# LiuShenLan/global_body_planner

Measured on AMD Instinct MI355X. Metric: valid extend-attempts/sec + time-to-first-solution, 1024×1024 rough_terrain, higher is better.
Workload: dtype f64; 1 GPU; config 3: synth-rough-1024, 262,144-attempt batch per GPU, isValidStateActionPair[Reverse] 50/50; terrain=synth-rough-1024, batch_per_gpu=262144, global_batch=262144, seed=20251018, kernel=persistent, waves=2, adaptive=False, terrain_storage=f32, parallelism=shard1 (no collective on the data path)

## Files before the change

global_body_planner_amd/csrc/gbp_engine.hip:

```cpp
#pragma clang fp contract(off)

#include <hip/hip_runtime.h>
#include <stdint.h>
#include <string.h>

#include <cstring>

#include <algorithm>
#include <cmath>
#include <mutex>
#include <new>
#include <vector>

#include "gbp.h"
#include "gbp_device.h"
#include "gbp_lane.h"
#include "gbp_um_order.h"
#include "gbp_internal.h"
#include "host/gbp_host_check.h"

using namespace gbp;

namespace {

// ... 53 lines not shown
    if (is_nan) is_nan[i] = r != 0 ? 1 : 0;
    if (ood) ood[i] = (!ok || r < 0) ? 1 : 0;
  }
}

template <class ZT>
__global__ void k_normal(TerrainView<ZT> T, int64_t n, const double *__restrict__ xy,
                         double *__restrict__ nrm, uint8_t *__restrict__ ood) {
  for (int64_t i = blockIdx.x * (int64_t)blockDim.x + threadIdx.x; i < n;
       i += (int64_t)gridDim.x * blockDim.x) {
    double v[3];
    const bool ok = surface_normal(T, xy[2 * i], xy[2 * i + 1], v);
    nrm[3 * i] = v[0];
    nrm[3 * i + 1] = v[1];
    nrm[3 * i + 2] = v[2];
    if (ood) ood[i] = ok ? 0 : 1;
  }
}

template <class ZT>
__global__ void k_valid_states(TerrainView<ZT> T, int64_t n, const double *__restrict__ states,
                               const uint8_t *__restrict__ phase, int phase_all,
                               uint8_t *__restrict__ valid, uint32_t *__restrict__ flags,
                               uint32_t *__restrict__ counts) {
  for (int64_t i = blockIdx.x * (int64_t)blockDim.x + threadIdx.x; i < n;
       i += (int64_t)gridDim.x * blockDim.x) {
    double s[8];
#pragma unroll
    for (int k = 0; k < 8; k++) s[k] = states[8 * i + k];
    Acc acc{0, 0, 0};
    const bool v = is_valid_state(T, s, phase ? phase[i] : phase_all, acc);
    if (valid) valid[i] = v;
    if (flags) flags[i] = acc.flags | (v ? GBP_F_VALID : 0u);
    if (counts) counts[i] = (acc.G & 0xFFFFu) | (acc.V << 16);
  }
}

extern __shared__ double gbp_smem[];

template <class ZT, bool ADAPTIVE, int W, int CM>
__global__ __launch_bounds__(256, W) void k_validate_direct(
    TerrainView<ZT> T0, int64_t n, const double *__restrict__ S, const double *__restrict__ A,
    const uint8_t *__restrict__ dir, int dir_all, uint8_t *__restrict__ valid,
    double *__restrict__ s_new, double *__restrict__ t_new, uint32_t *__restrict__ flags,
    uint32_t *__restrict__ counts) {
  const TerrainView<ZT> T = CM == 1 ? stage_coords(T0, gbp_smem) : T0;
  const int64_t i = blockIdx.x * (int64_t)blockDim.x + threadIdx.x;
  if (i >= n) return;
  double s[8], a[10], sn[8];
#pragma unroll
  for (int k = 0; k < 8; k++) s[k] = S[8 * i + k];
#pragma unroll
  for (int k = 0; k < 10; k++) a[k] = A[10 * i + k];
  double tn = 0;
  Acc acc{0, 0, 0};
  uint32_t f = 0;
  const int d = dir ? dir[i] : dir_all;
  const bool v = (d == GBP_FORWARD) ? pair_forward<ZT, ADAPTIVE>(T, s, a, sn, tn, acc, f)
                                    : pair_reverse<ZT, ADAPTIVE>(T, s, a, sn, tn, acc, f);
  f |= acc.flags | (v ? GBP_F_VALID : 0u);
  if (valid) valid[i] = v;
  if (s_new && (f & GBP_F_SNEW_SET)) {
#pragma unroll
    for (int k = 0; k < 8; k++) s_new[8 * i + k] = sn[k];
  }
  if (t_new && (f & GBP_F_TNEW_SET)) t_new[i] = tn;
  flags[i] = f;
  if (counts) counts[i] = (acc.G & 0xFFFFu) | (acc.V << 16);
}



struct SnewRec {
  int idx, kind;
  double p;
};
constexpr int SN_RING = 2 * 64;

#ifdef GBP_LOOP_PROF
constexpr int LP_N = 14;
__device__ unsigned long long gbp_loop_prof[8192 * LP_N];
#define LP_T(v) const unsigned long long v = __builtin_readcyclecounter()
#define LP_ADD(k, a, b) lp[k] += (b) - (a)
#else
#define LP_T(v)
#define LP_ADD(k, a, b)
#endif

[[maybe_unused]] constexpr int PF_MAX = 32;

inline size_t rows_bytes(int block, int pf) {
  const size_t nwv = (size_t)(block / WAVE);
  return sizeof(double) * SA_ROW * (size_t)(WAVE + pf) * nwv + sizeof(SnewRec) * SN_RING * nwv +
         sizeof(int) * ((nwv * (size_t)pf + 1) & ~(size_t)1);
}

__device__ __forceinline__ void row_to_lds(const double *S, const double *A, const uint8_t *dir,
                                           unsigned int i, double *row, int lane) {
  const unsigned int lds = __builtin_amdgcn_readfirstlane(
      (unsigned int)(uintptr_t)(__attribute__((address_space(3))) void *)row);
  const uint32_t *src = lane < 16 ? (const uint32_t *)(S + 8 * (size_t)i) + lane
                                  : (const uint32_t *)(A + 10 * (size_t)i) + (lane - 16);
  unsigned int keep;
  if (lane < 36)
    asm volatile("s_mov_b32 %0, m0\n\ts_mov_b32 m0, %2\n\ts_nop 0\n\t"
                 "global_load_lds_dword %1, off\n\ts_mov_b32 m0, %0"
                 : "=&s"(keep) : "v"(src), "s"(lds) : "memory");
  if (dir && lane == 36)
    asm volatile("s_mov_b32 %0, m0\n\ts_mov_b32 m0, %2\n\ts_nop 0\n\t"
                 "global_load_lds_ubyte %1, off\n\ts_mov_b32 m0, %0"
                 : "=&s"(keep) : "v"(dir + i), "s"(lds) : "memory");
}

template <class ZT, bool ADAPTIVE, int W, int CM, bool ONE>
__global__ __launch_bounds__(512, W) void k_validate_persistent(
    TerrainView<ZT> T0, int n, const double *__restrict__ S, const double *__restrict__ A,
    const uint8_t *__restrict__ dir, int dir_all, uint8_t *__restrict__ valid,
    double *__restrict__ s_new, double *__restrict__ t_new, uint32_t *__restrict__ flags,
    uint32_t *__restrict__ counts, const int *__restrict__ n_dev, int helpers, int xcd_map, int pf) {
#ifdef GBP_LOOP_PROF
  const unsigned long long lp_entry = __builtin_amdgcn_s_memrealtime();
#endif
  if (n_dev) n = *n_dev;
  const int lane = threadIdx.x & (WAVE - 1);
  const unsigned long long lt_mask = (1ull << lane) - 1ull;
  const int nwv = blockDim.x / WAVE, wv = __builtin_amdgcn_readfirstlane(threadIdx.x / WAVE);
  double *const SA = gbp_smem + (CM == 1 ? (T0.nx + T0.ny + 1) & ~1 : 0);
  double *const wave_rows = SA + (size_t)wv * (WAVE + pf) * SA_ROW;
  SnewRec *const ring = (SnewRec *)(SA + (size_t)nwv * (WAVE + pf) * SA_ROW) + wv * SN_RING;
  [[maybe_unused]] int *const Q = (int *)(ring + (nwv - wv) * SN_RING) + wv * pf;
  unsigned int cur, end;
  {
    const unsigned int waves = gridDim.x * (blockDim.x / WAVE);
    const unsigned int wg = (xcd_map && (gridDim.x & 7u) == 0)
                                ? (blockIdx.x & 7u) * (gridDim.x >> 3) + (blockIdx.x >> 3)
                                : blockIdx.x;
    const unsigned int wid = wg * (blockDim.x / WAVE) + wv;
    cur = __builtin_amdgcn_readfirstlane((unsigned int)(((unsigned long long)n * wid) / waves));
    end = __builtin_amdgcn_readfirstlane((unsigned int)(((unsigned long long)n * (wid + 1)) / waves));
  }
  auto load_row = [&](unsigned int i, double *r, int &d) {
    if (dir) d = dir[i];
#pragma unroll
    for (int k = 0; k < 8; k++) r[k] = S[8 * (size_t)i + k];
#pragma unroll
    for (int k = 0; k < 10; k++) r[8 + k] = A[10 * (size_t)i + k];
  };
#ifdef GBP_REFILL_WINDOW
  const unsigned int take0 = min(end - cur, (unsigned int)WAVE);
  double row0[18];
  int dir0 = dir_all;
  if ((unsigned int)lane < take0) load_row(cur + lane, row0, dir0);
#endif
  const TerrainView<ZT> T = CM == 1 ? stage_coords(T0, gbp_smem) : T0;
  int ring_n = 0;
  auto flush = [&](int cnt) {
    if (lane < cnt) {
      const SnewRec r = ring[lane];
      double sv[8], av[10], o[8];
#pragma unroll
      for (int k = 0; k < 8; k++) sv[k] = S[8 * (size_t)r.idx + k];
#pragma unroll
      for (int k = 0; k < 10; k++) av[k] = A[10 * (size_t)r.idx + k];
      sample_state(sv, av,
                   r.kind == SN_STANCE_S ? ST_FWD_STANCE
                                         : (r.kind == SN_FLIGHT_B ? ST_FWD_LAND : ST_REV_STANCE),
                   r.p, o);
#pragma unroll
      for (int k = 0; k < 8; k++) s_new[8 * (size_t)r.idx + k] = o[k];
    }
  };
  Lane L;
  int row = lane;
  L.s = wave_rows + row * SA_ROW;
  L.a = L.s + 8;
  L.stage = ST_IDLE;
  auto start = [&](unsigned int i, int d) {
    L.idx = (int)i;
    L.f = 0;
    L.acc = Acc{0, 0, 0};
    L.snew_kind = SN_NONE;
    L.tnew_set = 0;
    enter_stage(L, d == GBP_FORWARD ? ST_FWD_STANCE : ST_REV_FLIGHT);
  };
#ifdef GBP_REFILL_WINDOW
  unsigned int staged = 0, qh = 0;
  if (lane < pf) Q[lane] = WAVE + lane;
  if ((unsigned int)lane < take0) {
#pragma unroll
    for (int k = 0; k < 18; k++) L.s[k] = row0[k];
    start(cur + lane, dir0);
  }
  cur += take0;
#endif
#ifdef GBP_LOOP_PROF
  unsigned long long lp[LP_N] = {0, 0, 0, 0, 0, 0, 0, 0, 0, 0, 0, 0, 0, 0};
  lp[12] = lp_entry;
  lp[8] = __builtin_amdgcn_s_memrealtime();
  LP_T(lp_start);
#endif
  for (;;) {
    LP_T(t0);
    const bool need = L.stage == ST_IDLE;
    unsigned long long m = __ballot(need);
    if (m && cur < end) {
      const unsigned int take = min(end - cur, (unsigned int)__popcll(m));
      const unsigned int rank = (unsigned int)__popcll(m & lt_mask);
      const bool mine = need && rank < take;
      unsigned int ts = 0;
#ifdef GBP_REFILL_WINDOW
      ts = min(take, staged);
      if (ts) {
        asm volatile("s_waitcnt vmcnt(0)" ::: "memory");
        if (mine && rank < ts) {
          unsigned int p = qh + rank;
          p -= p >= (unsigned int)pf ? (unsigned int)pf : 0u;
          const int got = Q[p];
          Q[p] = row;
          row = got;
          L.s = wave_rows + row * SA_ROW;
          L.a = L.s + 8;
          start(cur + rank, dir ? ((const int *)L.s)[36] & 0xFF : dir_all);
        }
        qh += ts;
        qh -= qh >= (unsigned int)pf ? (unsigned int)pf : 0u;
        staged -= ts;
      }
#endif
      if (mine && rank >= ts) {
        double r[18];
        int d = dir_all;
        load_row(cur + rank, r, d);
#pragma unroll
        for (int k = 0; k < 18; k++) L.s[k] = r[k];
        start(cur + rank, d);
      }
      cur += take;
    }
#ifdef GBP_REFILL_WINDOW
    if (pf && min(end - cur, (unsigned int)pf) > staged) {
      const unsigned int want = min(end - cur, (unsigned int)pf);
      const int qv = Q[lane < pf ? lane : 0];
      for (unsigned int k = staged; k < want; k++) {
        unsigned int p = qh + k;
        p -= p >= (unsigned int)pf ? (unsigned int)pf : 0u;
        row_to_lds(S, A, dir, cur + k, wave_rows + __builtin_amdgcn_readlane(qv, p) * SA_ROW, lane);
      }
      staged = want;
    }
#endif
    const unsigned long long act = __ballot(L.stage != ST_IDLE);
    if (!act) break;
    LP_T(t1);
    LP_ADD(0, t0, t1);
#ifdef GBP_LOOP_PROF
    if (!lp[7]) lp[13] = __builtin_amdgcn_s_memrealtime();
#endif
    const bool owner = L.stage != ST_IDLE;
    asm volatile("" ::: "memory");
    const int n_act = __popcll(act);
    const bool tail = helpers && n_act < WAVE;
    int st = L.stage, slot = 0;
    const double *ps = L.s;
    double t_eval = owner ? stage_time(L) : 0.0;
    uint32_t vbase = L.acc.V;
    bool has = owner;
    if (tail) {
      const unsigned long long idle = ~act;
      const int j = __popcll(idle & lt_mask);
      const int src = owner ? lane : nth_set_bit(act, j % n_act);
      slot = owner ? 0 : 1 + j / n_act;
      ps = wave_rows + __shfl(row, src) * SA_ROW;
      st = __shfl(L.stage, src);
      double t = __shfl(L.t, src), ts = __shfl(L.ts, src);
      vbase = __shfl(L.acc.V, src);
      if (!owner) {
        has = true;
        for (int k = 0; k < slot && has; k++) has = advance_on_success<ADAPTIVE>(st, ps + 8, t, ts);
        t_eval = sample_time(st, ps + 8, t);
      }
    }
    LP_T(t2);
    LP_ADD(1, t1, t2);
    Acc acc_s{0, vbase + (uint32_t)slot, 0};
    bool ok = false;
    if (has) {
      double sc[8];
      sample_state(ps, ps + 8, st, t_eval, sc);
      ok = is_valid_state<ZT, CM, ONE>(T, sc, stage_phase(st), acc_s);
    }
    LP_T(t3);
    LP_ADD(2, t2, t3);
    bool decided = false;
    if (owner) {
      L.acc.G += acc_s.G;
      L.acc.V = acc_s.V;
      L.acc.flags |= acc_s.flags;
      decided = (acc_s.flags & GBP_F_LIMIT) ? true : transition<ADAPTIVE>(L, ok);
    }
    if (tail) {
      const unsigned long long idle = ~act;
      const int n_idle = WAVE - n_act;
      const int n_help = n_idle;
      const uint32_t w0 = (acc_s.flags & 0xFFFFu) | (ok ? 1u << 16 : 0u) | (has ? 1u << 17 : 0u) |
                          ((acc_s.V - (vbase + (uint32_t)slot)) << 18);
      const uint32_t w1 = acc_s.G;
      const int my_rank = __popcll(act & lt_mask);
      bool chain = owner && !decided && ok;
      const int kmax = (n_help + n_act - 1) / n_act;
      for (int k = 1; k <= kmax; k++) {
        if (!__ballot(chain)) break;
        const int j = (k - 1) * n_act + my_rank;
        const bool exists = owner && j < n_help;
        const int src = (exists && j < n_idle) ? nth_set_bit(idle, j) : lane;
        const uint32_t r0 = __shfl(w0, src), r1 = __shfl(w1, src);
        if (chain && exists && ((r0 >> 17) & 1u)) {
          L.acc.G += r1;
          L.acc.V += (r0 >> 18) & 1u;
          L.acc.flags |= r0 & 0xFFFFu;
          const bool okk = (r0 >> 16) & 1u;
          decided = (r0 & GBP_F_LIMIT) ? true : transition<ADAPTIVE>(L, okk);
          chain = !decided && okk;
        } else {
          chain = false;
        }
      }
    }
    asm volatile("" ::: "memory");
    LP_T(t4);
    LP_ADD(3, t3, t4);
#ifdef GBP_LOOP_PROF
    lp[6] += tail ? 1 : 0;
    lp[7] += 1;
#endif
    const bool fin = owner && decided;
    const bool queue = fin && s_new && L.snew_kind != SN_NONE;
    if (fin) {
      const size_t i = (size_t)L.idx;
      uint32_t f = L.f | L.acc.flags;
      if (L.snew_kind != SN_NONE) f |= GBP_F_SNEW_SET;
      if (L.tnew_set) f |= GBP_F_TNEW_SET;
      if (valid) valid[i] = (f & GBP_F_VALID) ? 1 : 0;
      if (t_new && L.tnew_set) t_new[i] = L.tnew;
      flags[i] = f;
      if (counts) counts[i] = (L.acc.G & 0xFFFFu) | (L.acc.V << 16);
    }
    const unsigned long long qm = __ballot(queue);
    if (qm) {
      if (queue) ring[ring_n + __popcll(qm & lt_mask)] = SnewRec{L.idx, L.snew_kind, L.snew_p};
      ring_n += __popcll(qm);
      if (ring_n >= WAVE) {
        flush(WAVE);
        ring_n -= WAVE;
        SnewRec r;
        if (lane < ring_n) r = ring[WAVE + lane];
        if (lane < ring_n) ring[lane] = r;
      }
    }
    if (fin) L.stage = ST_IDLE;
    LP_T(t5);
    LP_ADD(4, t4, t5);
  }
  if (ring_n) flush(ring_n);
#ifdef GBP_LOOP_PROF
  LP_T(lp_end);
  lp[5] = lp_end - lp_start;
  lp[9] = __builtin_amdgcn_s_memrealtime();
  {
    unsigned int hw;
    asm volatile("s_getreg_b32 %0, hwreg(HW_REG_HW_ID)" : "=s"(hw));
    lp[10] = hw;
    unsigned int xcc;
    asm volatile("s_getreg_b32 %0, hwreg(HW_REG_XCC_ID)" : "=s"(xcc));
    lp[11] = xcc;
  }
  const unsigned int gw = blockIdx.x * (blockDim.x / WAVE) + threadIdx.x / WAVE;
  if (lane == 0 && gw < 8192)
    for (int k = 0; k < LP_N; k++) gbp_loop_prof[LP_N * gw + k] = lp[k];
#endif
}

struct DirPair {
  double from[8], to[8];
};

template <class ZT>
__global__ void k_sample_states(TerrainView<ZT> T, int64_t n, uint64_t seed, uint64_t stream_id,
                                int64_t index_base, int require_phase, int max_tries,
                                double *__restrict__ states, int32_t *__restrict__ tries,
                                gbp_sampling cfg, DirPair dp) {
  for (int64_t i = blockIdx.x * (int64_t)blockDim.x + threadIdx.x; i < n;
       i += (int64_t)gridDim.x * blockDim.x) {
    double q[8];
    int got = -1;
    const int mt = max_tries > 0 ? max_tries : 1;
    for (int k = 0; k < mt; k++) {
      sample_state_cfg_try(T, cfg, dp.from, dp.to, seed, stream_id, index_base + i, k, q);
      if (require_phase < 0) { got = k + 1; break; }
      Acc acc{0, 0, 0};
      if (is_valid_state(T, q, require_phase, acc)) { got = k + 1; break; }
    }
#pragma unroll
    for (int k = 0; k < 8; k++) states[8 * i + k] = q[k];
    if (tries) tries[i] = got;
  }
}

__global__ void k_sample_actions(int64_t n, const double *__restrict__ normals, uint64_t seed,
                                 uint64_t stream_id, int64_t index_base,
                                 double *__restrict__ actions) {
  for (int64_t i = blockIdx.x * (int64_t)blockDim.x + threadIdx.x; i < n;
       i += (int64_t)gridDim.x * blockDim.x) {
    const double nv[3] = {normals[3 * i], normals[3 * i + 1], normals[3 * i + 2]};
    double a[10];
    sample_action(nv, seed, stream_id, index_base + i, a);
#pragma unroll
    for (int k = 0; k < 10; k++) actions[10 * i + k] = a[k];
  }
}

__global__ void k_sample_actions_dir(int64_t n, const double *__restrict__ normals,
                                     const double *__restrict__ s, const double *__restrict__ s_near,
                                     const uint8_t *__restrict__ dir, int dir_all, gbp_sampling cfg,
                                     uint64_t seed, uint64_t stream_id, int64_t index_base,
                                     double *__restrict__ actions) {
  for (int64_t i = blockIdx.x * (int64_t)blockDim.x + threadIdx.x; i < n;
       i += (int64_t)gridDim.x * blockDim.x) {
    const double nv[3] = {normals[3 * i], normals[3 * i + 1], normals[3 * i + 2]};
    double a[10];
    sample_action_cfg(nv, cfg, dir ? dir[i] : dir_all, s + 8 * i, s_near + 8 * i, seed, stream_id,
                      index_base + i, a);
#pragma unroll
    for (int k = 0; k < 10; k++) actions[10 * i + k] = a[k];
  }
}

template <class ZT>
__global__ void k_extend_prep(TerrainView<ZT> T, int64_t n, const double *__restrict__ s_near,
                              const double *__restrict__ target, const uint8_t *__restrict__ dir,
                              int dir_all, uint64_t seed, int64_t extend_base,
                              double *__restrict__ cand_s, double *__restrict__ cand_a,
                              uint8_t *__restrict__ cand_dir, gbp_sampling cfg) {
  const int64_t m = n * GBP_NUM_GEN_STATES;
  for (int64_t c = blockIdx.x * (int64_t)blockDim.x + threadIdx.x; c < m;
// ... 200 lines not shown
  return da < db || (da == db && ia < ib);
}
__device__ __forceinline__ void knn_cx(double &kd, int &ki, double &od, int j, bool lo) {
  const double pd = __shfl_xor(kd, j);
  const int pi = __shfl_xor(ki, j);
  const double po = __shfl_xor(od, j);
  const bool take = lo ? knn_less(pd, pi, kd, ki) : knn_less(kd, ki, pd, pi);
  if (take) {
    kd = pd;
    ki = pi;
    od = po;
  }
}

template <bool YAW>
__global__ __launch_bounds__(256) void k_knn(int64_t n_query, const double *__restrict__ q,
                                             int64_t n_vert, const double *__restrict__ v, int nk,
                                             int32_t *__restrict__ out, double *__restrict__ dist,
                                             const double *__restrict__ qyaw,
                                             const double *__restrict__ vyaw, double lw, double yw) {
  const int lane = threadIdx.x & (WAVE - 1);
  const int64_t waves = (int64_t)gridDim.x * (blockDim.x / WAVE);
  for (int64_t qi = blockIdx.x * (int64_t)(blockDim.x / WAVE) + threadIdx.x / WAVE; qi < n_query;
       qi += waves) {
    double qq[8];
#pragma unroll
    for (int k = 0; k < 8; k++) qq[k] = q[8 * qi + k];
    double kd = INFINITY, od = __builtin_nan("");
    int ki = 0x7FFFFFFF;
    for (int64_t j0 = 0; j0 < n_vert; j0 += WAVE) {
      const int64_t j = j0 + lane;
      double cd = INFINITY, co = __builtin_nan("");
      int ci = 0x7FFFFFFF;
      if (j < n_vert) {
        if constexpr (YAW)
          co = pose_distance(qq, v + 8 * j) * lw + yaw_distance(qyaw[qi], vyaw[j]) * yw;
        else
          co = state_distance(qq, v + 8 * j);
        cd = isnan(co) ? INFINITY : co;
        ci = (int)j;
      }
      const double td = __shfl(kd, nk - 1);
      const int ti = __shfl(ki, nk - 1);
      if (!__ballot(knn_less(cd, ci, td, ti))) continue;
#pragma unroll
      for (int k = 2; k <= WAVE; k <<= 1)
#pragma unroll
        for (int jj = k >> 1; jj > 0; jj >>= 1) {
          const bool up = (lane & k) == 0;
          knn_cx(cd, ci, co, jj, ((lane & jj) == 0) == up);
        }
      {
        const double rd = __shfl(cd, WAVE - 1 - lane);
        const int ri = __shfl(ci, WAVE - 1 - lane);
        const double ro = __shfl(co, WAVE - 1 - lane);
        if (knn_less(rd, ri, kd, ki)) {
          kd = rd;
          ki = ri;
          od = ro;
        }
      }
#pragma unroll
      for (int jj = WAVE >> 1; jj > 0; jj >>= 1) knn_cx(kd, ki, od, jj, (lane & jj) == 0);
    }
    if (lane < nk) {
      const bool real = ki != 0x7FFFFFFF;
      out[qi * nk + lane] = real ? ki : -1;
      if (dist) dist[qi * nk + lane] = real ? od : __builtin_nan("");
    }
  }
}

}

namespace {

int coord_mode(const gbp_terrain *t, bool lds_ok) {
  if (lds_ok) return 1;
  return (t->opt_affine && t->affine) ? 2 : 0;
}

int validate_block(const gbp_terrain *t, bool n_dev) {
  if (t->opt_block) return (int)t->opt_block;
  const size_t wg = stage_bytes(t->nx, t->ny) + rows_bytes(128, 0);
  if (!n_dev && (size_t)t->opt_waves * 2 * wg <= 160 * 1024) return 128;
  return 256;
}

int validate_coord_mode(const gbp_terrain *t, bool direct, bool n_dev = false) {
  const int block = validate_block(t, n_dev);
  const size_t rows = direct ? 0 : rows_bytes(block, 0);
  const size_t per_cu = std::max<int64_t>(1, t->opt_waves * 256 / block) *
                        (stage_bytes(t->nx, t->ny) + rows);
  const bool lds_ok = t->opt_lds_coords && stage_bytes(t->nx, t->ny) + rows <= t->lds_max &&
                      (direct || per_cu <= 160 * 1024);
  if (!direct && !(t->one_x && t->one_y)) return 0;
  return coord_mode(t, lds_ok);
}

int refill_window(const gbp_terrain *t, size_t coords, bool n_dev = false) {
#ifndef GBP_REFILL_WINDOW
  return 0;
#else
  const int block = validate_block(t, n_dev);
  const size_t wgs = (size_t)std::max<int64_t>(1, t->opt_waves * 256 / block);
  const size_t cap = std::min<size_t>(t->lds_max, 160 * 1024 / wgs);
  for (int pf = PF_MAX; pf > 0; pf--)
    if (coords + rows_bytes(block, pf) <= cap) return pf;
  return 0;
#endif
}

template <class ZT, bool AD, int W, int CM, bool ONE>
int launch_validate_w(gbp_terrain *t, int64_t n, const double *s, const double *a,
                      const uint8_t *dir, int dir_all, uint8_t *valid, double *s_new,
                      double *t_new, uint32_t *flags, uint32_t *counts, hipStream_t st,
                      const int *n_dev) {
  const TerrainView<ZT> T = view<ZT>(t);
  const int block = validate_block(t, n_dev != nullptr);
  const size_t coords = CM == 1 ? stage_bytes(t->nx, t->ny) : 0;
  const int64_t chunk = (int64_t)1 << 30;
  for (int64_t off = 0; off < n; off += chunk) {
    const int64_t m = std::min<int64_t>(n - off, chunk);
    const uint8_t *d = dir ? dir + off : nullptr;
    uint8_t *v = valid ? valid + off : nullptr;
    double *sn = s_new ? s_new + 8 * off : nullptr;
    double *tn = t_new ? t_new + off : nullptr;
    uint32_t *c = counts ? counts + off : nullptr;
    if (t->opt_kernel == GBP_KERNEL_DIRECT && !n_dev) {
      const int db = t->opt_block ? std::min(block, 256) : 256;
      const unsigned g = (unsigned)((m + db - 1) / db);
      hipLaunchKernelGGL((k_validate_direct<ZT, AD, 1, CM == 2 ? 0 : CM>), dim3(g), dim3(db), coords, st, T, m,
                         s + 8 * off, a + 10 * off, d, dir_all, v, sn, tn, flags + off, c);
    } else {
      const int64_t resident = (int64_t)t->num_cus * std::max<int64_t>(1, t->opt_waves * 256 / block);
      const int64_t g = std::max<int64_t>(1, std::min<int64_t>(resident, (m + WAVE - 1) / WAVE));
      const int pf = refill_window(t, coords, n_dev != nullptr);
      hipLaunchKernelGGL((k_validate_persistent<ZT, AD, W, CM, ONE>), dim3((unsigned)g), dim3(block),
                         coords + rows_bytes(block, pf), st, T, (int)m, s + 8 * off, a + 10 * off, d, dir_all,
                         v, sn, tn, flags + off, c, n_dev, (int)t->opt_helpers, (int)t->opt_xcd_map, pf);
    }
    HIPCHK(hipGetLastError());
  }
  return GBP_OK;
}

template <class ZT>
int launch_validate(gbp_terrain *t, int64_t n, const double *s, const double *a,
                    const uint8_t *dir, int dir_all, int adaptive, uint8_t *valid,
                    double *s_new, double *t_new, uint32_t *flags, uint32_t *counts,
                    hipStream_t st, const int *n_dev = nullptr) {
#define GBP_LVW(AD, W, CM, ONE)                                                              \
  launch_validate_w<ZT, AD, W, CM, ONE>(t, n, s, a, dir, dir_all, valid, s_new, t_new, flags,  \
                                        counts, st, n_dev)
#define GBP_LV(AD, W)                                                                        \
  (cm == 2 ? GBP_LVW(AD, W, 2, true)                                                         \
   : cm == 1 ? GBP_LVW(AD, W, 1, true)                                                       \
             : (one ? GBP_LVW(AD, W, 0, true) : GBP_LVW(AD, W, 0, false)))
  const int64_t w = t->opt_waves;
  const int cm = validate_coord_mode(t, t->opt_kernel == GBP_KERNEL_DIRECT && !n_dev, n_dev != nullptr);
  const bool one = t->one_x && t->one_y;
  if (adaptive) return w >= 4 ? GBP_LV(true, 4) : (w == 3 ? GBP_LV(true, 3) : GBP_LV(true, 2));
  return w >= 4 ? GBP_LV(false, 4) : (w == 3 ? GBP_LV(false, 3) : GBP_LV(false, 2));
#undef GBP_LV
#undef GBP_LVW
}

bool valid_handle(const gbp_terrain *t) { return t != nullptr && t->d_z != nullptr; }

int guess_host(int n, double d0, double inv, double v) {
  const int i = (int)((v - d0) * inv);
  return i < 0 ? 0 : (i > n - 2 ? n - 2 : i);
}

int one_step_exact(const double *d, int n, double inv) {
  if (!(inv > 0) || !std::isfinite(inv)) return 0;
  for (int i = 0; i + 1 < n; i++) {
    if (!(d[i] < d[i + 1])) return 0;
    const int lo = guess_host(n, d[0], inv, d[i]);
    const int hi = guess_host(n, d[0], inv, std::nextafter(d[i + 1], -INFINITY));
    if (lo < i - 1 || hi > i + 1) return 0;
  }
  return 1;
}

bool affine_exact(const double *d, int n, double a, double h, int base) {
  for (int i = 0; i < n; i++) {
    const double v = a + h * (double)(i - base);
    if (memcmp(&v, &d[i], sizeof v) != 0) return false;
  }
  return true;
}

double verified_rcp_seed(const double *x, int nx, const double *y, int ny) {
  if (nx < 2 || ny < 2) return 0.0;
  auto spacings = [](const double *d, int n) {
    std::vector<double> v;
    for (int i = 0; i + 1 < n; i++) v.push_back(d[i + 1] - d[i]);
    std::sort(v.begin(), v.end());
    v.erase(std::unique(v.begin(), v.end(), [](double a, double b) {
              return memcmp(&a, &b, sizeof a) == 0;
            }), v.end());
    return v;
  };
  const std::vector<double> sx = spacings(x, nx), sy = spacings(y, ny);
  if ((double)sx.size() * (double)sy.size() > 4e6) return 0.0;
  const double seed = 1.0 / (((x[nx - 1] - x[0]) / (double)(nx - 1)) *
                             ((y[ny - 1] - y[0]) / (double)(ny - 1)));
  if (!std::isfinite(seed) || !(seed > 0)) return 0.0;
  for (double dx : sx)
    for (double dy : sy) {
      const double d = dx * dy;
      const double q = 1.0 / d, r = recip_newton(d, seed);
      if (memcmp(&q, &r, sizeof q) != 0) return 0.0;
    }
  return seed;
}

bool affine_fit(const double *d, int n, double *a, double *h, int *base) {
  if (n < 2) return false;
  const double cands[3] = {(d[n - 1] - d[0]) / (double)(n - 1), d[1] - d[0], d[n - 1] - d[n - 2]};
  for (int b = 0; b < 2; b++) {
    const int bs = b ? n - 1 : 0;
    const double av = d[bs];
    for (double c : cands) {
      if (!(c > 0) || !std::isfinite(c)) continue;
      double hv = c;
      for (int k = 0; k < 4; k++) hv = std::nextafter(hv, -INFINITY);
      for (int k = 0; k < 9; k++, hv = std::nextafter(hv, INFINITY)) {
        if (affine_exact(d, n, av, hv, bs)) {
          *a = av;
          *h = hv;
          *base = bs;
          return true;
        }
      }
    }
  }
  return false;
}

template <class F>
int stage_ws(gbp_terrain *t, F carve) {
  const int rc = ensure_ws(&t->ws, &t->ws_bytes, stage_bytes_of(carve));
  return rc ? rc : stage_carve(t->ws, t->ws_bytes, carve);
}

}

__attribute__((visibility("hidden"))) int gbp_internal_validate_dev_n(
    gbp_terrain *t, int64_t n_max, const int *n_dev, const double *s, const double *a,
    const uint8_t *dir, int dir_all, int adaptive, uint8_t *valid, double *s_new, double *t_new,
    uint32_t *flags, uint32_t *counts, hipStream_t st) {
  if (n_max <= 0) return GBP_OK;
  if (t->storage == GBP_STORAGE_F32)
    return launch_validate<float>(t, n_max, s, a, dir, dir_all, adaptive, valid, s_new, t_new,
                                  flags, counts, st, n_dev);
  return launch_validate<double>(t, n_max, s, a, dir, dir_all, adaptive, valid, s_new, t_new,
                                 flags, counts, st, n_dev);
}

extern "C" {

#ifdef GBP_LOOP_PROF
int gbp_loop_prof_read(unsigned long long *out, int n_waves) {
  if (!out || n_waves < 0 || n_waves > 8192) return GBP_E_INVALID_ARG;
  if (hipDeviceSynchronize() != hipSuccess) return GBP_E_HIP;
  if (hipMemcpyFromSymbol(out, HIP_SYMBOL(gbp_loop_prof), sizeof(unsigned long long) * LP_N * n_waves) !=
      hipSuccess)
    return GBP_E_HIP;
  return GBP_OK;
}
#endif

int gbp_validate_lds_plan(int nx, int ny, int64_t block, int64_t waves, size_t lds_max,
                          int *coord_lds, int *window, size_t *bytes) {
  if (nx < 2 || ny < 2 || (block && block < WAVE) || block > 512 || block % WAVE || waves < 1)
    return GBP_E_INVALID_ARG;
  gbp_terrain t;
  t.nx = nx;
  t.ny = ny;
  t.one_x = t.one_y = 1;
  t.opt_affine = 0;
  t.opt_block = block;
  t.opt_waves = waves;
  t.lds_max = lds_max;
  const int cm = validate_coord_mode(&t, false);
  const size_t coords = cm == 1 ? stage_bytes(nx, ny) : 0;
  const int pf = refill_window(&t, coords);
  if (coord_lds) *coord_lds = cm == 1;
  if (window) *window = pf;
  if (bytes) *bytes = coords + rows_bytes(validate_block(&t, false), pf);
  return GBP_OK;
}

int gbp_version(void) { return 200;  }

const char *gbp_status_string(int status) {
  switch (status) {
    case GBP_OK: return "ok";
    case GBP_E_INVALID_ARG: return "invalid argument";
    case GBP_E_BAD_HANDLE: return "bad handle";
    case GBP_E_ALLOC: return "device allocation failed";
    case GBP_E_HIP: return "HIP runtime error";
    case GBP_E_SHAPE: return "bad shape";
    case GBP_E_NO_DEVICE: return "no HIP device";
    case GBP_E_UNSUPPORTED: return "unsupported";
    default: return "unknown status";
  }
}

int gbp_device_count(int *count) {
  if (!count) return GBP_E_INVALID_ARG;
  int c = 0;
  if (hipGetDeviceCount(&c) != hipSuccess) c = 0;
  *count = c;
  return c > 0 ? GBP_OK : GBP_E_NO_DEVICE;
}

int gbp_device_alloc(int device, size_t bytes, void **ptr) {
  if (!ptr) return GBP_E_INVALID_ARG;
  DeviceGuard g(device);
  if (hipMalloc(ptr, bytes ? bytes : 1) != hipSuccess) return GBP_E_ALLOC;
  return GBP_OK;
}

int gbp_device_free(void *ptr) {
  if (ptr) HIPCHK(hipFree(ptr));
  return GBP_OK;
}

int gbp_memcpy_h2d(void *dst, const void *src, size_t bytes, gbp_stream stream) {
  HIPCHK(hipMemcpyAsync(dst, src, bytes, hipMemcpyHostToDevice, (hipStream_t)stream));
  return GBP_OK;
}

int gbp_memcpy_d2h(void *dst, const void *src, size_t bytes, gbp_stream stream) {
  HIPCHK(hipMemcpyAsync(dst, src, bytes, hipMemcpyDeviceToHost, (hipStream_t)stream));
  return GBP_OK;
}

int gbp_stream_synchronize(gbp_stream stream) {
  HIPCHK(hipStreamSynchronize((hipStream_t)stream));
  return GBP_OK;
}

int gbp_terrain_create(int device, int nx, int ny, const double *x, const double *y,
                       const double *z, const double *dx, const double *dy, const double *dz,
                       int storage, gbp_terrain **out) {
  if (!out || !x || !y || !z) return GBP_E_INVALID_ARG;
  *out = nullptr;
  if (nx < 2 || ny < 2) return GBP_E_SHAPE;
  if ((dx == nullptr) != (dy == nullptr) || (dx == nullptr) != (dz == nullptr))
    return GBP_E_INVALID_ARG;
  for (int i = 0; i + 1 < nx; i++)
    if (!(x[i] <= x[i + 1])) return GBP_E_INVALID_ARG;
  for (int i = 0; i + 1 < ny; i++)
    if (!(y[i] <= y[i + 1])) return GBP_E_INVALID_ARG;
  const size_t cells = (size_t)nx * ny;
  if (storage == GBP_STORAGE_AUTO) {
    storage = GBP_STORAGE_F32;
    for (size_t i = 0; i < cells; i++) {
      const double v = z[i];
      if (!std::isnan(v) && (double)(float)v != v) {
        storage = GBP_STORAGE_F64;
        break;
      }
    }
  } else if (storage != GBP_STORAGE_F32 && storage != GBP_STORAGE_F64) {
    return GBP_E_INVALID_ARG;
  }
  int ndev = 0;
  if (hipGetDeviceCount(&ndev) != hipSuccess || ndev == 0) return GBP_E_NO_DEVICE;
  if (device < 0 || device >= ndev) return GBP_E_INVALID_ARG;
  DeviceGuard g(device);
// ... 84 lines not shown
  (void)hipDeviceSynchronize();
  void *ptrs[] = {t->d_x, t->d_y, t->d_z, t->d_dx, t->d_dy, t->d_dz, t->ws};
  for (void *p : ptrs)
    if (p) (void)hipFree(p);
  for (auto &w : t->cand_ws)
    if (w.ptr) (void)hipFree(w.ptr);
  for (auto &u : t->pending) (void)hipEventDestroy(u.done);
  if (t->host_stream) (void)hipStreamDestroy(t->host_stream);
  delete t;
  return GBP_OK;
}

int gbp_terrain_info(const gbp_terrain *t, int *nx, int *ny, int *storage, double bounds[4],
                     int *device) {
  if (!valid_handle(t)) return GBP_E_BAD_HANDLE;
  if (nx) *nx = t->nx;
  if (ny) *ny = t->ny;
  if (storage) *storage = t->storage;
  if (bounds) memcpy(bounds, t->bounds, sizeof t->bounds);
  if (device) *device = t->device;
  return GBP_OK;
}

int gbp_terrain_set_option(gbp_terrain *t, int key, int64_t value) {
  if (!valid_handle(t)) return GBP_E_BAD_HANDLE;
  switch (key) {
    case GBP_OPT_KERNEL:
      if (value != GBP_KERNEL_DIRECT && value != GBP_KERNEL_PERSISTENT) return GBP_E_INVALID_ARG;
      t->opt_kernel = value;
      return GBP_OK;
    case GBP_OPT_BLOCK:
      if (value && (value < 64 || value > 512 || value % 64)) return GBP_E_INVALID_ARG;
      t->opt_block = value;
      return GBP_OK;
    case GBP_OPT_WAVES:
      if (value < 1 || value > 4) return GBP_E_INVALID_ARG;
      t->opt_waves = value;
      return GBP_OK;
    case GBP_OPT_LDS_COORDS:
      t->opt_lds_coords = value ? 1 : 0;
      return GBP_OK;
    case GBP_OPT_HELPERS:
      t->opt_helpers = value ? 1 : 0;
      return GBP_OK;
    case GBP_OPT_AFFINE_COORDS:
      t->opt_affine = value ? 1 : 0;
      return GBP_OK;
    case GBP_OPT_XCD_MAP:
      t->opt_xcd_map = value ? 1 : 0;
      return GBP_OK;
    case GBP_OPT_FAST_RCP:
      t->opt_fast_rcp = value ? 1 : 0;
      return GBP_OK;
    case GBP_OPT_NN_STATS:
      t->opt_nn_stats = value ? 1 : 0;
      return GBP_OK;
    case GBP_OPT_FRAGILE_EPS:
      if (value < 1000 || value > 1000000000000000LL) return GBP_E_INVALID_ARG;
      t->fragile_eps = (double)value * 1e-15;
      return GBP_OK;
    default:
      return GBP_E_INVALID_ARG;
  }
}

int gbp_terrain_get_option(const gbp_terrain *t, int key, int64_t *value) {
  if (!valid_handle(t)) return GBP_E_BAD_HANDLE;
  if (!value) return GBP_E_INVALID_ARG;
  switch (key) {
    case GBP_OPT_KERNEL: *value = t->opt_kernel; return GBP_OK;
    case GBP_OPT_BLOCK: *value = t->opt_block ? t->opt_block : 256; return GBP_OK;
    case GBP_OPT_LAUNCH_BLOCK: *value = validate_block(t, false); return GBP_OK;
    case GBP_OPT_WAVES: *value = t->opt_waves; return GBP_OK;
    case GBP_OPT_LDS_COORDS: *value = t->opt_lds_coords; return GBP_OK;
    case GBP_OPT_HELPERS: *value = t->opt_helpers; return GBP_OK;
    case GBP_OPT_AFFINE_COORDS: *value = t->opt_affine; return GBP_OK;
    case GBP_OPT_XCD_MAP: *value = t->opt_xcd_map; return GBP_OK;
    case GBP_OPT_FAST_RCP: *value = t->opt_fast_rcp ? (t->rcp_seed != 0.0 ? 1 : 0) : 0; return GBP_OK;
    case GBP_OPT_NN_STATS: *value = t->opt_nn_stats; return GBP_OK;
    case GBP_OPT_FRAGILE_EPS: *value = (int64_t)std::llround(t->fragile_eps * 1e15); return GBP_OK;
    case GBP_OPT_COORD_MODE:
      *value = validate_coord_mode(t, t->opt_kernel == GBP_KERNEL_DIRECT);
      return GBP_OK;
    case GBP_OPT_REFILL_WINDOW:
      *value = refill_window(t, validate_coord_mode(t, false) == 1 ? stage_bytes(t->nx, t->ny) : 0);
      return GBP_OK;
    default: return GBP_E_INVALID_ARG;
  }
}

int gbp_height_batch_dev(gbp_terrain *t, int64_t n, const double *xy, double *height,
                         uint8_t *is_nan, uint8_t *ood, gbp_stream stream) {
  if (!valid_handle(t)) return GBP_E_BAD_HANDLE;
  if (n < 0 || (n > 0 && !xy)) return GBP_E_INVALID_ARG;
  if (n == 0) return GBP_OK;
  DeviceGuard g(t->device);
  if (((uintptr_t)xy) % 16) return GBP_E_INVALID_ARG;
  const size_t cbytes = stage_bytes(t->nx, t->ny);
  const bool lds = t->opt_lds_coords && cbytes <= t->lds_max;
  const unsigned grid = grid_for(n, 256, t->num_cus * 8);
  const double2 *p = (const double2 *)xy;
  hipStream_t st = (hipStream_t)stream;
  const int cm = coord_mode(t, lds);
#define GBP_K1(ZT, CM)                                                                      \
  hipLaunchKernelGGL((k_height<ZT, CM>), dim3(grid), dim3(256), CM == 1 ? cbytes : 0, st, \
                     view<ZT>(t), n, p, height, is_nan, ood)
  if (t->storage == GBP_STORAGE_F32) {
    if (cm == 2) GBP_K1(float, 2);
    else if (cm == 1) GBP_K1(float, 1);
    else GBP_K1(float, 0);
  } else {
    if (cm == 2) GBP_K1(double, 2);
    else if (cm == 1) GBP_K1(double, 1);
    else GBP_K1(double, 0);
  }
#undef GBP_K1
  HIPCHK(hipGetLastError());
  return GBP_OK;
}

int gbp_normal_batch_dev(gbp_terrain *t, int64_t n, const double *xy, double *normal,
                         uint8_t *ood, gbp_stream stream) {
  if (!valid_handle(t)) return GBP_E_BAD_HANDLE;
  if (n < 0 || (n > 0 && (!xy || !normal))) return GBP_E_INVALID_ARG;
  if (n == 0) return GBP_OK;
  DeviceGuard g(t->device);
  const unsigned grid = grid_for(n, 256, t->num_cus * 16);
  if (t->storage == GBP_STORAGE_F32)
    hipLaunchKernelGGL(k_normal<float>, dim3(grid), dim3(256), 0, (hipStream_t)stream,
                       view<float>(t), n, xy, normal, ood);
  else
    hipLaunchKernelGGL(k_normal<double>, dim3(grid), dim3(256), 0, (hipStream_t)stream,
                       view<double>(t), n, xy, normal, ood);
  HIPCHK(hipGetLastError());
  return GBP_OK;
}

int gbp_valid_states_dev(gbp_terrain *t, int64_t n, const double *states, const uint8_t *phase,
                         int phase_all, uint8_t *valid, uint32_t *flags, uint32_t *counts,
                         gbp_stream stream) {
  if (!valid_handle(t)) return GBP_E_BAD_HANDLE;
  if (n < 0 || (n > 0 && !states)) return GBP_E_INVALID_ARG;
  if (n == 0) return GBP_OK;
  DeviceGuard g(t->device);
  const unsigned grid = grid_for(n, 256, t->num_cus * 16);
  if (t->storage == GBP_STORAGE_F32)
    hipLaunchKernelGGL(k_valid_states<float>, dim3(grid), dim3(256), 0, (hipStream_t)stream,
                       view<float>(t), n, states, phase, phase_all, valid, flags, counts);
  else
    hipLaunchKernelGGL(k_valid_states<double>, dim3(grid), dim3(256), 0, (hipStream_t)stream,
                       view<double>(t), n, states, phase, phase_all, valid, flags, counts);
  HIPCHK(hipGetLastError());
  return GBP_OK;
}

int gbp_validate_pairs_dev(gbp_terrain *t, int64_t n, const double *s, const double *a,
                           const uint8_t *direction, int direction_all, int adaptive,
                           uint8_t *valid, double *s_new, double *t_new, uint32_t *flags,
                           uint32_t *counts, gbp_stream stream) {
  if (!valid_handle(t)) return GBP_E_BAD_HANDLE;
  if (n < 0 || (n > 0 && (!s || !a || !flags))) return GBP_E_INVALID_ARG;
  if (!direction && direction_all != GBP_FORWARD && direction_all != GBP_REVERSE)
    return GBP_E_INVALID_ARG;
  if (n == 0) return GBP_OK;
  DeviceGuard g(t->device);
  if (t->storage == GBP_STORAGE_F32)
    return launch_validate<float>(t, n, s, a, direction, direction_all, adaptive, valid, s_new,
                                  t_new, flags, counts, (hipStream_t)stream);
  return launch_validate<double>(t, n, s, a, direction, direction_all, adaptive, valid, s_new,
// ... 681 lines not shown
```

Measured before the change: 2.965 billion extend-attempts/s.

## Replace LDS refill window with register-prefetched row ring and deferred output writes

Removes the compile-time-disabled LDS refill window, which used global_load_lds with a queue of row slots. In its place, each lane prefetches its next work row (S, A, dir) into registers during the step loop and scatters it with ds_permute into the LDS row of the lane that picks up that index. The per-lane result stores and s_new ring handling move to the top of the next iteration, so their latency overlaps the refill. The goal is to hide global-load latency for new work items. The cost is 18 extra doubles of registers per lane, and the path is only enabled for f32 terrain with W<=2 and large batches.

```diff
diff --git a/global_body_planner_amd/csrc/gbp_engine.hip b/global_body_planner_amd/csrc/gbp_engine.hip
--- a/global_body_planner_amd/csrc/gbp_engine.hip
+++ b/global_body_planner_amd/csrc/gbp_engine.hip
@@ -159,42 +159,27 @@
 __device__ unsigned long long gbp_loop_prof[8192 * LP_N];
 #define LP_T(v) const unsigned long long v = __builtin_readcyclecounter()
 #define LP_ADD(k, a, b) lp[k] += (b) - (a)
+#define LP_DO(x) x
 #else
 #define LP_T(v)
 #define LP_ADD(k, a, b)
+#define LP_DO(x)
 #endif
 
-[[maybe_unused]] constexpr int PF_MAX = 32;
-
-inline size_t rows_bytes(int block, int pf) {
+inline size_t rows_bytes(int block) {
   const size_t nwv = (size_t)(block / WAVE);
-  return sizeof(double) * SA_ROW * (size_t)(WAVE + pf) * nwv + sizeof(SnewRec) * SN_RING * nwv +
-         sizeof(int) * ((nwv * (size_t)pf + 1) & ~(size_t)1);
-}
-
-__device__ __forceinline__ void row_to_lds(const double *S, const double *A, const uint8_t *dir,
-                                           unsigned int i, double *row, int lane) {
-  const unsigned int lds = __builtin_amdgcn_readfirstlane(
-      (unsigned int)(uintptr_t)(__attribute__((address_space(3))) void *)row);
-  const uint32_t *src = lane < 16 ? (const uint32_t *)(S + 8 * (size_t)i) + lane
-                                  : (const uint32_t *)(A + 10 * (size_t)i) + (lane - 16);
-  unsigned int keep;
-  if (lane < 36)
-    asm volatile("s_mov_b32 %0, m0\n\ts_mov_b32 m0, %2\n\ts_nop 0\n\t"
-                 "global_load_lds_dword %1, off\n\ts_mov_b32 m0, %0"
-                 : "=&s"(keep) : "v"(src), "s"(lds) : "memory");
-  if (dir && lane == 36)
-    asm volatile("s_mov_b32 %0, m0\n\ts_mov_b32 m0, %2\n\ts_nop 0\n\t"
-                 "global_load_lds_ubyte %1, off\n\ts_mov_b32 m0, %0"
-                 : "=&s"(keep) : "v"(dir + i), "s"(lds) : "memory");
-}
-
-template <class ZT, bool ADAPTIVE, int W, int CM, bool ONE>
+  return sizeof(double) * SA_ROW * (size_t)WAVE * nwv + sizeof(SnewRec) * SN_RING * nwv;
+}
+
+template <class ZT, int W, int CM, bool ONE>
+constexpr bool refill_ring = W <= 2 && sizeof(ZT) == 4 && !(CM == 0 && ONE);
+
+template <class ZT, bool ADAPTIVE, int W, int CM, bool ONE, bool RING>
 __global__ __launch_bounds__(512, W) void k_validate_persistent(
     TerrainView<ZT> T0, int n, const double *__restrict__ S, const double *__restrict__ A,
     const uint8_t *__restrict__ dir, int dir_all, uint8_t *__restrict__ valid,
     double *__restrict__ s_new, double *__restrict__ t_new, uint32_t *__restrict__ flags,
-    uint32_t *__restrict__ counts, const int *__restrict__ n_dev, int helpers, int xcd_map, int pf) {
+    uint32_t *__restrict__ counts, const int *__restrict__ n_dev, int helpers, int xcd_map) {
 #ifdef GBP_LOOP_PROF
   const unsigned long long lp_entry = __builtin_amdgcn_s_memrealtime();
 #endif
@@ -203,9 +188,8 @@
   const unsigned long long lt_mask = (1ull << lane) - 1ull;
   const int nwv = blockDim.x / WAVE, wv = __builtin_amdgcn_readfirstlane(threadIdx.x / WAVE);
   double *const SA = gbp_smem + (CM == 1 ? (T0.nx + T0.ny + 1) & ~1 : 0);
-  double *const wave_rows = SA + (size_t)wv * (WAVE + pf) * SA_ROW;
-  SnewRec *const ring = (SnewRec *)(SA + (size_t)nwv * (WAVE + pf) * SA_ROW) + wv * SN_RING;
-  [[maybe_unused]] int *const Q = (int *)(ring + (nwv - wv) * SN_RING) + wv * pf;
+  double *const wave_rows = SA + (size_t)wv * WAVE * SA_ROW;
+  SnewRec *const ring = (SnewRec *)(SA + (size_t)nwv * WAVE * SA_ROW) + wv * SN_RING;
   unsigned int cur, end;
   {
     const unsigned int waves = gridDim.x * (blockDim.x / WAVE);
@@ -223,12 +207,12 @@
 #pragma unroll
     for (int k = 0; k < 10; k++) r[8 + k] = A[10 * (size_t)i + k];
   };
-#ifdef GBP_REFILL_WINDOW
-  const unsigned int take0 = min(end - cur, (unsigned int)WAVE);
-  double row0[18];
-  int dir0 = dir_all;
-  if ((unsigned int)lane < take0) load_row(cur + lane, row0, dir0);
-#endif
+  const unsigned int begin = cur;
+  [[maybe_unused]] double pr[18];
+  [[maybe_unused]] int pd = dir_all;
+  [[maybe_unused]] unsigned int nk = WAVE + lane;
+  [[maybe_unused]] bool held = false;
+  bool pend = false;
   const TerrainView<ZT> T = CM == 1 ? stage_coords(T0, gbp_smem) : T0;
   int ring_n = 0;
   auto flush = [&](int cnt) {
@@ -248,8 +232,7 @@
     }
   };
   Lane L;
-  int row = lane;
-  L.s = wave_rows + row * SA_ROW;
+  L.s = wave_rows + lane * SA_ROW;
   L.a = L.s + 8;
   L.stage = ST_IDLE;
   auto start = [&](unsigned int i, int d) {
@@ -260,76 +243,81 @@
     L.tnew_set = 0;
     enter_stage(L, d == GBP_FORWARD ? ST_FWD_STANCE : ST_REV_FLIGHT);
   };
-#ifdef GBP_REFILL_WINDOW
-  unsigned int staged = 0, qh = 0;
-  if (lane < pf) Q[lane] = WAVE + lane;
-  if ((unsigned int)lane < take0) {
-#pragma unroll
-    for (int k = 0; k < 18; k++) L.s[k] = row0[k];
-    start(cur + lane, dir0);
-  }
-  cur += take0;
-#endif
 #ifdef GBP_LOOP_PROF
   unsigned long long lp[LP_N] = {0, 0, 0, 0, 0, 0, 0, 0, 0, 0, 0, 0, 0, 0};
   lp[12] = lp_entry;
   lp[8] = __builtin_amdgcn_s_memrealtime();
   LP_T(lp_start);
+  unsigned long long lp_out = 0;
 #endif
+  auto put_outputs = [&]() {
+    LP_T(t0o);
+    const bool queue = pend && s_new && L.snew_kind != SN_NONE;
+    if (pend) {
+      const size_t i = (size_t)L.idx;
+      uint32_t f = L.f | L.acc.flags;
+      if (L.snew_kind != SN_NONE) f |= GBP_F_SNEW_SET;
+      if (L.tnew_set) f |= GBP_F_TNEW_SET;
+      if (valid) valid[i] = (f & GBP_F_VALID) ? 1 : 0;
+      if (t_new && L.tnew_set) t_new[i] = L.tnew;
+      flags[i] = f;
+      if (counts) counts[i] = (L.acc.G & 0xFFFFu) | (L.acc.V << 16);
+    }
+    pend = false;
+    const unsigned long long qm = __ballot(queue);
+    if (qm) {
+      if (queue) ring[ring_n + __popcll(qm & lt_mask)] = SnewRec{L.idx, L.snew_kind, L.snew_p};
+      ring_n += __popcll(qm);
+      if (ring_n >= WAVE) {
+        flush(WAVE);
+        ring_n -= WAVE;
+        SnewRec r;
+        if (lane < ring_n) r = ring[WAVE + lane];
+        if (lane < ring_n) ring[lane] = r;
+      }
+    }
+    LP_T(t1o);
+    LP_ADD(4, t0o, t1o);
+    LP_DO(lp_out = t1o - t0o);
+  };
   for (;;) {
     LP_T(t0);
     const bool need = L.stage == ST_IDLE;
-    unsigned long long m = __ballot(need);
-    if (m && cur < end) {
-      const unsigned int take = min(end - cur, (unsigned int)__popcll(m));
-      const unsigned int rank = (unsigned int)__popcll(m & lt_mask);
-      const bool mine = need && rank < take;
-      unsigned int ts = 0;
-#ifdef GBP_REFILL_WINDOW
-      ts = min(take, staged);
-      if (ts) {
-        asm volatile("s_waitcnt vmcnt(0)" ::: "memory");
-        if (mine && rank < ts) {
-          unsigned int p = qh + rank;
-          p -= p >= (unsigned int)pf ? (unsigned int)pf : 0u;
-          const int got = Q[p];
-          Q[p] = row;
-          row = got;
-          L.s = wave_rows + row * SA_ROW;
-          L.a = L.s + 8;
-          start(cur + rank, dir ? ((const int *)L.s)[36] & 0xFF : dir_all);
-        }
-        qh += ts;
-        qh -= qh >= (unsigned int)pf ? (unsigned int)pf : 0u;
-        staged -= ts;
+    const unsigned long long m = __ballot(need);
+    const unsigned int take = min(end - cur, (unsigned int)__popcll(m));
+    const unsigned int rank = (unsigned int)__popcll(m & lt_mask);
+    const bool mine = need && rank < take;
+    const bool from_ring = RING && take && cur != begin;
+    if (from_ring) {
+      const unsigned int r = nk - (cur - begin);
+      const int dest = __builtin_amdgcn_ds_permute((int)((cur - begin + (mine ? rank : take)) & 63u) << 2, lane);
+      if (held && r < take) {
+        double *const dst = wave_rows + dest * SA_ROW;
+#pragma unroll
+        for (int k = 0; k < 18; k++) dst[k] = pr[k];
+        if (dir) ((int *)dst)[36] = pd;
+        held = false;
+        nk += WAVE;
       }
-#endif
-      if (mine && rank >= ts) {
-        double r[18];
-        int d = dir_all;
-        load_row(cur + rank, r, d);
-#pragma unroll
-        for (int k = 0; k < 18; k++) L.s[k] = r[k];
-        start(cur + rank, d);
-      }
-      cur += take;
-    }
-#ifdef GBP_REFILL_WINDOW
-    if (pf && min(end - cur, (unsigned int)pf) > staged) {
-      const unsigned int want = min(end - cur, (unsigned int)pf);
-      const int qv = Q[lane < pf ? lane : 0];
-      for (unsigned int k = staged; k < want; k++) {
-        unsigned int p = qh + k;
-        p -= p >= (unsigned int)pf ? (unsigned int)pf : 0u;
-        row_to_lds(S, A, dir, cur + k, wave_rows + __builtin_amdgcn_readlane(qv, p) * SA_ROW, lane);
-      }
-      staged = want;
-    }
-#endif
+      asm volatile("" ::: "memory");
+    }
+    if (RING) put_outputs();
+    if (from_ring) {
+      if (mine) start(cur + rank, dir ? ((const int *)L.s)[36] & 0xFF : dir_all);
+    } else if (mine) {
+      double r[18];
+      int d = dir_all;
+      load_row(cur + rank, r, d);
+#pragma unroll
+      for (int k = 0; k < 18; k++) L.s[k] = r[k];
+      start(cur + rank, d);
+    }
+    cur += take;
     const unsigned long long act = __ballot(L.stage != ST_IDLE);
     if (!act) break;
     LP_T(t1);
     LP_ADD(0, t0, t1);
+    LP_DO(if (RING) lp[0] -= lp_out; lp_out = 0);
 #ifdef GBP_LOOP_PROF
     if (!lp[7]) lp[13] = __builtin_amdgcn_s_memrealtime();
 #endif
@@ -347,7 +335,7 @@
       const int j = __popcll(idle & lt_mask);
       const int src = owner ? lane : nth_set_bit(act, j % n_act);
       slot = owner ? 0 : 1 + j / n_act;
-      ps = wave_rows + __shfl(row, src) * SA_ROW;
+      ps = wave_rows + src * SA_ROW;
       st = __shfl(L.stage, src);
       double t = __shfl(L.t, src), ts = __shfl(L.ts, src);
       vbase = __shfl(L.acc.V, src);
@@ -368,6 +356,15 @@
     }
     LP_T(t3);
     LP_ADD(2, t2, t3);
+    if (RING && !held && nk < end - begin) {
+      const size_t i = begin + nk;
+#pragma unroll
+      for (int k = 0; k < 8; k++) pr[k] = S[8 * i + k];
+#pragma unroll
+      for (int k = 0; k < 10; k++) pr[8 + k] = A[10 * i + k];
+      if (dir) pd = dir[i];
+      held = true;
+    }
     bool decided = false;
     if (owner) {
       L.acc.G += acc_s.G;
@@ -411,32 +408,9 @@
     lp[7] += 1;
 #endif
     const bool fin = owner && decided;
-    const bool queue = fin && s_new && L.snew_kind != SN_NONE;
-    if (fin) {
-      const size_t i = (size_t)L.idx;
-      uint32_t f = L.f | L.acc.flags;
-      if (L.snew_kind != SN_NONE) f |= GBP_F_SNEW_SET;
-      if (L.tnew_set) f |= GBP_F_TNEW_SET;
-      if (valid) valid[i] = (f & GBP_F_VALID) ? 1 : 0;
-      if (t_new && L.tnew_set) t_new[i] = L.tnew;
-      flags[i] = f;
-      if (counts) counts[i] = (L.acc.G & 0xFFFFu) | (L.acc.V << 16);
-    }
-    const unsigned long long qm = __ballot(queue);
-    if (qm) {
-      if (queue) ring[ring_n + __popcll(qm & lt_mask)] = SnewRec{L.idx, L.snew_kind, L.snew_p};
-      ring_n += __popcll(qm);
-      if (ring_n >= WAVE) {
-        flush(WAVE);
-        ring_n -= WAVE;
-        SnewRec r;
-        if (lane < ring_n) r = ring[WAVE + lane];
-        if (lane < ring_n) ring[lane] = r;
-      }
-    }
+    pend = fin;
+    if (!RING) put_outputs();
     if (fin) L.stage = ST_IDLE;
-    LP_T(t5);
-    LP_ADD(4, t4, t5);
   }
   if (ring_n) flush(ring_n);
 #ifdef GBP_LOOP_PROF
@@ -803,33 +777,20 @@
 
 int validate_block(const gbp_terrain *t, bool n_dev) {
   if (t->opt_block) return (int)t->opt_block;
-  const size_t wg = stage_bytes(t->nx, t->ny) + rows_bytes(128, 0);
+  const size_t wg = stage_bytes(t->nx, t->ny) + rows_bytes(128);
   if (!n_dev && (size_t)t->opt_waves * 2 * wg <= 160 * 1024) return 128;
   return 256;
 }
 
 int validate_coord_mode(const gbp_terrain *t, bool direct, bool n_dev = false) {
   const int block = validate_block(t, n_dev);
-  const size_t rows = direct ? 0 : rows_bytes(block, 0);
+  const size_t rows = direct ? 0 : rows_bytes(block);
   const size_t per_cu = std::max<int64_t>(1, t->opt_waves * 256 / block) *
                         (stage_bytes(t->nx, t->ny) + rows);
   const bool lds_ok = t->opt_lds_coords && stage_bytes(t->nx, t->ny) + rows <= t->lds_max &&
                       (direct || per_cu <= 160 * 1024);
   if (!direct && !(t->one_x && t->one_y)) return 0;
   return coord_mode(t, lds_ok);
-}
-
-int refill_window(const gbp_terrain *t, size_t coords, bool n_dev = false) {
-#ifndef GBP_REFILL_WINDOW
-  return 0;
-#else
-  const int block = validate_block(t, n_dev);
-  const size_t wgs = (size_t)std::max<int64_t>(1, t->opt_waves * 256 / block);
-  const size_t cap = std::min<size_t>(t->lds_max, 160 * 1024 / wgs);
-  for (int pf = PF_MAX; pf > 0; pf--)
-    if (coords + rows_bytes(block, pf) <= cap) return pf;
-  return 0;
-#endif
 }
 
 template <class ZT, bool AD, int W, int CM, bool ONE>
@@ -856,10 +817,15 @@
     } else {
       const int64_t resident = (int64_t)t->num_cus * std::max<int64_t>(1, t->opt_waves * 256 / block);
       const int64_t g = std::max<int64_t>(1, std::min<int64_t>(resident, (m + WAVE - 1) / WAVE));
-      const int pf = refill_window(t, coords, n_dev != nullptr);
-      hipLaunchKernelGGL((k_validate_persistent<ZT, AD, W, CM, ONE>), dim3((unsigned)g), dim3(block),
-                         coords + rows_bytes(block, pf), st, T, (int)m, s + 8 * off, a + 10 * off, d, dir_all,
-                         v, sn, tn, flags + off, c, n_dev, (int)t->opt_helpers, (int)t->opt_xcd_map, pf);
+      constexpr bool CAN = refill_ring<ZT, W, CM, ONE>;
+      const bool ring = CAN && m > (int64_t)WAVE * g * (block / WAVE);
+      auto go = [&](auto kernel) {
+        hipLaunchKernelGGL(kernel, dim3((unsigned)g), dim3(block), coords + rows_bytes(block), st, T, (int)m,
+                           s + 8 * off, a + 10 * off, d, dir_all, v, sn, tn, flags + off, c, n_dev,
+                           (int)t->opt_helpers, (int)t->opt_xcd_map);
+      };
+      if (ring) go(k_validate_persistent<ZT, AD, W, CM, ONE, CAN>);
+      else go(k_validate_persistent<ZT, AD, W, CM, ONE, false>);
     }
     HIPCHK(hipGetLastError());
   }
@@ -1008,10 +974,9 @@
   t.lds_max = lds_max;
   const int cm = validate_coord_mode(&t, false);
   const size_t coords = cm == 1 ? stage_bytes(nx, ny) : 0;
-  const int pf = refill_window(&t, coords);
   if (coord_lds) *coord_lds = cm == 1;
-  if (window) *window = pf;
-  if (bytes) *bytes = coords + rows_bytes(validate_block(&t, false), pf);
+  if (window) *window = 0;
+  if (bytes) *bytes = coords + rows_bytes(validate_block(&t, false));
   return GBP_OK;
 }
 
@@ -1262,9 +1227,7 @@
     case GBP_OPT_COORD_MODE:
       *value = validate_coord_mode(t, t->opt_kernel == GBP_KERNEL_DIRECT);
       return GBP_OK;
-    case GBP_OPT_REFILL_WINDOW:
-      *value = refill_window(t, validate_coord_mode(t, false) == 1 ? stage_bytes(t->nx, t->ny) : 0);
-      return GBP_OK;
+    case GBP_OPT_REFILL_WINDOW: *value = 0; return GBP_OK;
     default: return GBP_E_INVALID_ARG;
   }
 }
```

After: 3.021 billion extend-attempts/s, median of 6. 1.02x the previous value.
